# Wangshihu12/colmap-pcd

Hardware: AMD Instinct MI355X
Metric: NN queries/sec + BA-iter ms, 10M-pt cloud / 1M 3D feats (higher is better)
Workload: dtype f32 (NN distances) / f64 (association, BA); 1 GPU; M: 10000000-pt 'planes' cloud / 1000000 queries + BA scene 1000 cams / 1000000 pts / 4721253 obs / 900000 lidar terms (OPENCV), the same total at every N; cloud_points=10000000, queries=1000000, queries_this_rank=1000000, parallelism=single GPU

## Files before the change

colmap-pcd_amd/csrc/ba.hip:

```cpp
#include <algorithm>
#include <chrono>
#include <cmath>
#include <limits>
#include <memory>
#include <numeric>

#include "ba_cam_jac.h"
#include "ba_math.h"
#include "common.h"

namespace pcd {

struct BaDev {
  const int* cam_model; const int* cam_off; const double* cam_params;
  const double* poses; const int* image_cam; const uint8_t* image_const_pose; const uint8_t* image_const_tvec;
  const double* points; const uint8_t* point_const;
  const int* obs_image; const int* obs_point; const double* obs_xy;
  const int* lidar_point; const double* lidar_abcd; const double* lidar_w;
  const int* pt_order;
  const uint32_t* slice_start;
  const int* sell_img;
  const double* sell_xy;
  const uint32_t* pt_lidar_start; const uint32_t* pt_lidar_list;
  const uint32_t* img_obs_start;
  const int* img_pt;
  const uint32_t* img_obs;
  const uint32_t* seg_img;
  const uint32_t* seg_begin;
  const uint32_t* img_seg_start;
  const uint8_t* cam_refine;
  const uint32_t* cam_img_start;
  const uint32_t* cam_img_list;
  int C;
  int cam_k;
  const double* img_xy;
  int I, P, nslices; uint64_t O, L;
  int loss_type; double loss_scale;
};

template <int MODEL>
__device__ __forceinline__ void eval_block(const BaDev& d, int im, const double X[3], double ox, double oy,
                                           ReprojBlock& b, double q[4]) {
  const double* pose = d.poses + 7 * (size_t)im;
  double t[3];
#pragma unroll
  for (int k = 0; k < 4; ++k) q[k] = pose[k];
#pragma unroll
  for (int k = 0; k < 3; ++k) t[k] = pose[4 + k];
  const int cm = d.image_cam[im];
  const int model = MODEL >= 0 ? MODEL : d.cam_model[cm];
  reproj_eval(model, d.cam_params + d.cam_off[cm], q, t, X, ox, oy, b);
}

template <int N>
__device__ __forceinline__ void wave_store_rows(double* __restrict__ out, uint64_t row0, int cnt, const double (&v)[N],
                                                double* __restrict__ lds) {
  static_assert(N % 2 == 0, "rows are moved in 16-byte units");
  const int lane = threadIdx.x & 63;
#pragma unroll
  for (int k = 0; k < N; ++k) lds[lane * N + k] = v[k];
  __builtin_amdgcn_fence(__ATOMIC_RELEASE, "workgroup");
  __builtin_amdgcn_wave_barrier();
  __builtin_amdgcn_fence(__ATOMIC_ACQUIRE, "workgroup");
  const double2* src = reinterpret_cast<const double2*>(lds);
  double2* dst = reinterpret_cast<double2*>(out + row0 * N);
  const int units = cnt * (N / 2);
#pragma unroll
  for (int j = 0; j < N / 2; ++j) {
    const int u = j * 64 + lane;
    if (u < units) dst[u] = src[u];
  }
  __builtin_amdgcn_fence(__ATOMIC_RELEASE, "workgroup");
  __builtin_amdgcn_wave_barrier();
}

template <int MODEL, bool BLOCKS>
__global__ __launch_bounds__(256) void k_ba_points(BaDev d, double* __restrict__ Hpt, double* __restrict__ gpt,
                                                   double* __restrict__ cost_partial) {
  __shared__ double s_half[2][64][9];
  const int sl = threadIdx.x >> 7, half = (threadIdx.x >> 6) & 1, lane = threadIdx.x & 63;
  const int slice = blockIdx.x * 2 + sl;
  const int t = slice * 64 + lane;
  double cost = 0.0;
  double H[6] = {0, 0, 0, 0, 0, 0}, g[3] = {0, 0, 0};
  int p = -1;
  bool cpt = true;
  double X[3] = {0, 0, 0};
  if (slice < d.nslices) {
    p = d.pt_order[t];
    const uint32_t s0 = d.slice_start[slice], s1 = d.slice_start[slice + 1];
    if (p >= 0) {
      X[0] = d.points[3 * (size_t)p]; X[1] = d.points[3 * (size_t)p + 1]; X[2] = d.points[3 * (size_t)p + 2];
      cpt = d.point_const && d.point_const[p];
    }
    for (uint32_t s = s0 + lane + 64u * half; s < s1; s += 128) {
      const int im = d.sell_img[s];
      if (im < 0) continue;
      ReprojBlock b;
      double q[4];
      eval_block<MODEL>(d, im, X, d.sell_xy[2 * (size_t)s], d.sell_xy[2 * (size_t)s + 1], b, q);
      double rho0, rho1;
      loss_eval(d.loss_type, d.loss_scale, b.r[0] * b.r[0] + b.r[1] * b.r[1], rho0, rho1);
      cost += 0.5 * rho0;
      if (BLOCKS && !cpt) {
        const double sr = sqrt(rho1);
        double J[6];
#pragma unroll
        for (int r = 0; r < 2; ++r)
#pragma unroll
          for (int k = 0; k < 3; ++k)
            J[3 * r + k] = sr * (b.M[3 * r] * b.D[k] + b.M[3 * r + 1] * b.D[3 + k] + b.M[3 * r + 2] * b.D[6 + k]);
        const double r0 = sr * b.r[0], r1 = sr * b.r[1];
        H[0] += J[0] * J[0] + J[3] * J[3]; H[1] += J[0] * J[1] + J[3] * J[4]; H[2] += J[0] * J[2] + J[3] * J[5];
        H[3] += J[1] * J[1] + J[4] * J[4]; H[4] += J[1] * J[2] + J[4] * J[5]; H[5] += J[2] * J[2] + J[5] * J[5];
        g[0] += J[0] * r0 + J[3] * r1; g[1] += J[1] * r0 + J[4] * r1; g[2] += J[2] * r0 + J[5] * r1;
      }
    }
  }
  if (BLOCKS && half == 1) {
#pragma unroll
    for (int k = 0; k < 6; ++k) s_half[sl][lane][k] = H[k];
#pragma unroll
    for (int k = 0; k < 3; ++k) s_half[sl][lane][6 + k] = g[k];
  }
  __syncthreads();
  if (half == 0 && slice < d.nslices) {
    if (BLOCKS) {
#pragma unroll
      for (int k = 0; k < 6; ++k) H[k] += s_half[sl][lane][k];
#pragma unroll
      for (int k = 0; k < 3; ++k) g[k] += s_half[sl][lane][6 + k];
    }
    if (p >= 0) {
      for (uint32_t e = d.pt_lidar_start[p]; e < d.pt_lidar_start[p + 1]; ++e) {
        const uint32_t l = d.pt_lidar_list[e];
        const double abcd[4] = {d.lidar_abcd[4 * (size_t)l], d.lidar_abcd[4 * (size_t)l + 1],
                                d.lidar_abcd[4 * (size_t)l + 2], d.lidar_abcd[4 * (size_t)l + 3]};
        double r, J[3];
        lidar_eval(X, abcd, d.lidar_w[l], 0, r, J);
        double rho0, rho1;
        loss_eval(d.loss_type, d.loss_scale, r * r, rho0, rho1);
        cost += 0.5 * rho0;
        if (BLOCKS && !cpt) {
          const double sr = sqrt(rho1);
          const double rc = sr * r;
          J[0] *= sr; J[1] *= sr; J[2] *= sr;
          H[0] += J[0] * J[0]; H[1] += J[0] * J[1]; H[2] += J[0] * J[2];
          H[3] += J[1] * J[1]; H[4] += J[1] * J[2]; H[5] += J[2] * J[2];
          g[0] += J[0] * rc; g[1] += J[1] * rc; g[2] += J[2] * rc;
        }
      }
      if (BLOCKS && Hpt) {
        double* h = Hpt + 9 * (size_t)p;
        h[0] = H[0]; h[1] = H[1]; h[2] = H[2]; h[3] = H[1]; h[4] = H[3]; h[5] = H[4]; h[6] = H[2]; h[7] = H[4]; h[8] = H[5];
      }
      if (BLOCKS && gpt) { gpt[3 * (size_t)p] = g[0]; gpt[3 * (size_t)p + 1] = g[1]; gpt[3 * (size_t)p + 2] = g[2]; }
    }
  }
  __syncthreads();
  __shared__ double s_c[256];
  s_c[threadIdx.x] = cost;
  __syncthreads();
  for (int off = 128; off > 0; off >>= 1) {
    if ((int)threadIdx.x < off) s_c[threadIdx.x] += s_c[threadIdx.x + off];
    __syncthreads();
  }
  if (threadIdx.x == 0) cost_partial[blockIdx.x] = s_c[0];
}

template <int MODEL>
__global__ __launch_bounds__(256) void k_ba_cost(BaDev d, double* __restrict__ cost_partial) {
  double cost = 0.0;
  for (uint64_t i = blockIdx.x * (uint64_t)256 + threadIdx.x; i < d.O + d.L; i += (uint64_t)gridDim.x * 256) {
    if (i < d.O) {
      const int im = d.obs_image[i], pt = d.obs_point[i];
      const double X[3] = {d.points[3 * (size_t)pt], d.points[3 * (size_t)pt + 1], d.points[3 * (size_t)pt + 2]};
      ReprojBlock b;
      double q[4];
      eval_block<MODEL>(d, im, X, d.obs_xy[2 * i], d.obs_xy[2 * i + 1], b, q);
      double rho0, rho1;
      loss_eval(d.loss_type, d.loss_scale, b.r[0] * b.r[0] + b.r[1] * b.r[1], rho0, rho1);
      cost += 0.5 * rho0;
    } else {
      const uint64_t l = i - d.O;
      const int pt = d.lidar_point[l];
      const double X[3] = {d.points[3 * (size_t)pt], d.points[3 * (size_t)pt + 1], d.points[3 * (size_t)pt + 2]};
      const double abcd[4] = {d.lidar_abcd[4 * l], d.lidar_abcd[4 * l + 1], d.lidar_abcd[4 * l + 2], d.lidar_abcd[4 * l + 3]};
      double r, J[3];
      lidar_eval(X, abcd, d.lidar_w[l], 0, r, J);
      double rho0, rho1;
      loss_eval(d.loss_type, d.loss_scale, r * r, rho0, rho1);
      cost += 0.5 * rho0;
    }
  }
  __shared__ double s_c[256];
  s_c[threadIdx.x] = cost;
  __syncthreads();
  for (int off = 128; off > 0; off >>= 1) {
    if ((int)threadIdx.x < off) s_c[threadIdx.x] += s_c[threadIdx.x + off];
    __syncthreads();
  }
  if (threadIdx.x == 0) cost_partial[blockIdx.x] = s_c[0];
}
constexpr unsigned kCostBlocks = 1u << 20;

__global__ __launch_bounds__(256) void k_sum_partials(const double* __restrict__ partial, int n, double* __restrict__ out) {
  __shared__ double s_c[256];
  double a0 = 0.0, a1 = 0.0, a2 = 0.0, a3 = 0.0;
  int i = threadIdx.x;
  for (; i + 768 < n; i += 1024) { a0 += partial[i]; a1 += partial[i + 256]; a2 += partial[i + 512]; a3 += partial[i + 768]; }
  for (; i < n; i += 256) a0 += partial[i];
  s_c[threadIdx.x] = (a0 + a1) + (a2 + a3);
  __syncthreads();
  for (int off = 128; off > 0; off >>= 1) {
    if ((int)threadIdx.x < off) s_c[threadIdx.x] += s_c[threadIdx.x + off];
    __syncthreads();
  }
  if (threadIdx.x == 0) out[0] = s_c[0];
}

constexpr uint32_t kImgSeg = 1024;
template <int MODEL, bool WANT_W>
__global__ __launch_bounds__(256) void k_ba_images(BaDev d, double* __restrict__ partial, double* __restrict__ W_o) {
  __shared__ __attribute__((aligned(16))) double s_w[WANT_W ? 4 : 1][WANT_W ? 64 * 18 : 2];
  const int im = (int)d.seg_img[blockIdx.x];
  const int lane = threadIdx.x & 63;
  const int wave = __builtin_amdgcn_readfirstlane((int)(threadIdx.x >> 6));
  const bool cpose = d.image_const_pose && d.image_const_pose[im];
  double acc[27];
#pragma unroll
  for (int k = 0; k < 27; ++k) acc[k] = 0.0;
  const unsigned tmask = d.image_const_tvec ? d.image_const_tvec[im] : 0u;
  const uint32_t e_beg = d.seg_begin[blockIdx.x];
  const uint32_t e_end = min(d.seg_begin[blockIdx.x + 1], d.img_obs_start[im + 1]);
  if (!cpose || WANT_W) {
    for (uint32_t e0 = e_beg; e0 < e_end; e0 += 256) {
      const uint32_t e = e0 + threadIdx.x;
      const bool active = e < e_end;
      double w[18];
#pragma unroll
      for (int k = 0; k < 18; ++k) w[k] = 0.0;
      if (active && !cpose) {
        const int pt = d.img_pt[e];
        const double X[3] = {d.points[3 * (size_t)pt], d.points[3 * (size_t)pt + 1], d.points[3 * (size_t)pt + 2]};
        ReprojBlock b;
        double q[4];
        eval_block<MODEL>(d, im, X, d.img_xy[2 * (size_t)e], d.img_xy[2 * (size_t)e + 1], b, q);
        double rho0, rho1;
        loss_eval(d.loss_type, d.loss_scale, b.r[0] * b.r[0] + b.r[1] * b.r[1], rho0, rho1);
        const double sr = sqrt(rho1);
        double Jq[8], Jt[6], JX[6], Jqt[6];
        reproj_jacobians(b, Jq, Jt, JX);
        quat_tangent(q, Jq, Jqt);
        double J[12];
#pragma unroll
        for (int r = 0; r < 2; ++r)
#pragma unroll
          for (int k = 0; k < 3; ++k) {
            J[6 * r + k] = sr * Jqt[3 * r + k];
            J[6 * r + 3 + k] = ((tmask >> k) & 1u) ? 0.0 : sr * Jt[3 * r + k];
          }
        const double r0 = sr * b.r[0], r1 = sr * b.r[1];
        int idx = 0;
#pragma unroll
        for (int a = 0; a < 6; ++a)
#pragma unroll
          for (int c = a; c < 6; ++c) acc[idx++] += J[a] * J[c] + J[6 + a] * J[6 + c];
#pragma unroll
        for (int a = 0; a < 6; ++a) acc[21 + a] += J[a] * r0 + J[6 + a] * r1;
        if (WANT_W && !(d.point_const && d.point_const[pt])) {
#pragma unroll
          for (int a = 0; a < 6; ++a)
#pragma unroll
            for (int c = 0; c < 3; ++c) w[3 * a + c] = J[a] * (sr * JX[c]) + J[6 + a] * (sr * JX[3 + c]);
        }
      }
      if (WANT_W) {
        const uint32_t o = active ? d.img_obs[e] : 0u;
        const uint32_t o_first = (uint32_t)__builtin_amdgcn_readfirstlane((int)o);
        const int cnt = (int)min(64u, e_end > e0 + wave * 64u ? e_end - (e0 + wave * 64u) : 0u);
        const bool contiguous = __all(!active || o == o_first + (uint32_t)lane);
        if (contiguous) {
          wave_store_rows<18>(W_o, o_first, cnt, w, s_w[wave]);
        } else if (active) {
          double* dst = W_o + 18 * (size_t)o;
#pragma unroll
          for (int k = 0; k < 18; ++k) dst[k] = w[k];
        }
      }
    }
  }
  __shared__ double s_a[4][27];
#pragma unroll
  for (int k = 0; k < 27; ++k) {
    double v = acc[k];
#pragma unroll
    for (int off = 32; off > 0; off >>= 1) v += __shfl_xor(v, off);
    if (lane == 0) s_a[wave][k] = v;
  }
  __syncthreads();
  if (threadIdx.x < 27)
    partial[27 * (size_t)blockIdx.x + threadIdx.x] =
        (s_a[0][threadIdx.x] + s_a[1][threadIdx.x]) + (s_a[2][threadIdx.x] + s_a[3][threadIdx.x]);
}

__global__ __launch_bounds__(64) void k_ba_images_reduce(BaDev d, const double* __restrict__ partial,
                                                         double* __restrict__ Himg, double* __restrict__ gimg) {
  const int im = blockIdx.x * 2 + (threadIdx.x >> 5), k = threadIdx.x & 31;
  if (im >= d.I || k >= 27) return;
  double v = 0.0;
  for (uint32_t sgm = d.img_seg_start[im]; sgm < d.img_seg_start[im + 1]; ++sgm) v += partial[27 * (size_t)sgm + k];
  if (k >= 21) {
    if (gimg) gimg[6 * (size_t)im + (k - 21)] = v;
  } else if (Himg) {
    int a = 0, kk = k;
    while (kk >= 6 - a) { kk -= 6 - a; ++a; }
    const int c = a + kk;
    Himg[36 * (size_t)im + 6 * a + c] = v;
    Himg[36 * (size_t)im + 6 * c + a] = v;
  }
}

__host__ __device__ constexpr int cam_ne(int K) { return K * (K + 1) / 2 + 6 * K + K; }
__host__ __device__ constexpr int cam_ent_l(int K, int e) {
  const int ncc = K * (K + 1) / 2;
  if (e < ncc) { int a = 0; while (e >= K - a) { e -= K - a; ++a; } return a; }
  e -= ncc;
  if (e < 6 * K) return e / 6;
  return e - 6 * K;
}
__host__ __device__ constexpr int cam_ent_r(int K, int e) {
  const int ncc = K * (K + 1) / 2;
  if (e < ncc) { int a = 0; while (e >= K - a) { e -= K - a; ++a; } return a + e; }
  e -= ncc;
  if (e < 6 * K) return K + e % 6;
  return K + 6;
}

template <int MODEL, int CH>
__device__ __forceinline__ void cam_accumulate(const BaDev& d, int im, double* __restrict__ partial) {
  constexpr int K = MODEL >= 0 ? cam_num_params(MODEL >= 0 ? MODEL : 0) : PCD_CAM_JAC_STRIDE;
  constexpr int NE = cam_ne(K), PER = (NE + 3) / 4, E0 = CH * PER, E1 = E0 + PER < NE ? E0 + PER : NE;
  constexpr int NA = K + 7;
  const int lane = threadIdx.x & 63;
  const bool cpose = d.image_const_pose && d.image_const_pose[im];
  const unsigned tmask = d.image_const_tvec ? d.image_const_tvec[im] : 0u;
  const int cm = d.image_cam[im];
  const double* cam = d.cam_params + d.cam_off[cm];
  const uint8_t* refine = d.cam_refine ? d.cam_refine + d.cam_off[cm] : nullptr;
  const int model = MODEL >= 0 ? MODEL : d.cam_model[cm];
  double acc[PER > 0 ? PER : 1];
#pragma unroll
  for (int t = 0; t < PER; ++t) acc[t] = 0.0;
  for (uint32_t e = d.img_obs_start[im] + lane; e < d.img_obs_start[im + 1]; e += 64) {
    const int pt = d.img_pt[e];
    const double X[3] = {d.points[3 * (size_t)pt], d.points[3 * (size_t)pt + 1], d.points[3 * (size_t)pt + 2]};
    ReprojBlock b;
    double q[4];
    eval_block<MODEL>(d, im, X, d.img_xy[2 * (size_t)e], d.img_xy[2 * (size_t)e + 1], b, q);
    double rho0, rho1;
    loss_eval(d.loss_type, d.loss_scale, b.r[0] * b.r[0] + b.r[1] * b.r[1], rho0, rho1);
    const double sr = sqrt(rho1);
    double A[2][NA];
    {
      const double* pose = d.poses + 7 * (size_t)im;
      const double w = pose[0], a = pose[1], bq = pose[2], c = pose[3];
      const double cx = bq * X[2] - c * X[1], cy = c * X[0] - a * X[2], cz = a * X[1] - bq * X[0];
      const double ux = 2.0 * cx, uy = 2.0 * cy, uz = 2.0 * cz;
      const double Px = X[0] + w * ux + (bq * uz - c * uy) + pose[4];
      const double Py = X[1] + w * uy + (c * ux - a * uz) + pose[5];
      const double Pz = X[2] + w * uz + (a * uy - bq * ux) + pose[6];
      const double iz = 1.0 / Pz;
      double Jc[2 * K];
#pragma unroll
      for (int k = 0; k < 2 * K; ++k) Jc[k] = 0.0;
      if (MODEL >= 0) cam_param_jacobian<(MODEL >= 0 ? MODEL : 0)>(cam, Px * iz, Py * iz, Jc, K);
      else cam_param_jacobian_any(model, cam, Px * iz, Py * iz, Jc, K);
      const int kn = MODEL >= 0 ? K : cam_num_params(model);
#pragma unroll
      for (int k = 0; k < K; ++k) {
        const bool var = refine && k < kn && refine[k < kn ? k : 0];
        A[0][k] = var ? sr * Jc[k] : 0.0;
        A[1][k] = var ? sr * Jc[K + k] : 0.0;
      }
    }
    double Jq[8], Jt[6], JX[6], Jqt[6];
    reproj_jacobians(b, Jq, Jt, JX);
    quat_tangent(q, Jq, Jqt);
#pragma unroll
    for (int r = 0; r < 2; ++r) {
// ... 1332 lines not shown
      b->nseg = (uint32_t)seg_img.size();
      seg_begin.push_back((uint32_t)b->O);
      UP(seg_img, seg_img.data(), seg_img.size());
      UP(seg_begin, seg_begin.data(), seg_begin.size());
      UP(img_seg_start, img_seg_start.data(), img_seg_start.size());
    }
    {
      std::vector<uint32_t> cst, cli;
      build_csr(d->image_camera, (uint64_t)b->I, b->C, cst, cli);
      UP(cam_img_start, cst.data(), cst.size());
      UP(cam_img_list, cli.data(), cli.size());
    }
    UP(img_obs, li.data(), li.size());
    pcd_status sa = b->img_pt.reserve(std::max<size_t>(b->O, 1));
    if (sa == PCD_OK) sa = b->img_xy.reserve(std::max<size_t>(2 * b->O, 2));
    if (sa != PCD_OK) return fail(sa);
    if (b->O)
      hipLaunchKernelGGL(k_ba_fill_image_major, dim3(div_up(b->O, 256)), dim3(256), 0, nullptr, b->img_obs.p,
                         b->obs_point.p, b->obs_xy.p, b->O, b->img_pt.p, b->img_xy.p);
    if (hipDeviceSynchronize() != hipSuccess || hipGetLastError() != hipSuccess) {
      set_error("pcd_ba_create: filling the image-major layout failed");
      return fail(PCD_ERR_HIP);
    }
  }
#undef UP
  {
    b->h_pose_row.assign(b->O, 0xFFFFFFFFu);
    std::vector<uint32_t> vobs;
    vobs.reserve(b->O);
    for (uint64_t o = 0; o < b->O; ++o)
      if (!(d->image_const_pose && d->image_const_pose[d->obs_image[o]])) {
        b->h_pose_row[o] = (uint32_t)vobs.size();
        vobs.push_back((uint32_t)o);
      }
    b->n_pose_rows = vobs.size();
    if (b->n_pose_rows != b->O) {
      pcd_status sv = upload(b->vobs, vobs.data(), vobs.size());
      if (sv != PCD_OK) return fail(sv);
    }
  }
  pcd_status s1 = b->cost_partial.reserve((size_t)std::max(cost_blocks(b, true), cost_blocks(b, false)) + 1);
  if (s1 != PCD_OK) return fail(s1);
  if ((s1 = b->cost.reserve(1)) != PCD_OK) return fail(s1);
  *out = b;
  return PCD_OK;
  });
}

void pcd_ba_destroy(pcd_ba* b) {
  if (!b) return;
  (void)hipSetDevice(b->device);
  delete b;
}

pcd_status pcd_ba_set_parameters(pcd_ba* b, const double* poses, const double* points) {
  PCD_REQUIRE(b, "null handle");
  PCD_HIP_TRY(hipSetDevice(b->device));
  if (poses) PCD_HIP_TRY(hipMemcpy(b->poses.p, poses, 7 * (size_t)b->I * sizeof(double), hipMemcpyHostToDevice));
  if (points) PCD_HIP_TRY(hipMemcpy(b->points.p, points, 3 * (size_t)b->P * sizeof(double), hipMemcpyHostToDevice));
  return PCD_OK;
}

pcd_status pcd_ba_set_camera_parameters(pcd_ba* b, const double* cam_params) {
  PCD_REQUIRE(b && cam_params, "null pointer");
  PCD_HIP_TRY(hipSetDevice(b->device));
  PCD_HIP_TRY(hipMemcpy(b->cam_params.p, cam_params, b->cam_params_len * sizeof(double), hipMemcpyHostToDevice));
  return PCD_OK;
}

pcd_status pcd_ba_device_parameters(pcd_ba* b, double** d_poses, double** d_points) {
  PCD_REQUIRE(b, "null handle");
  if (d_poses) *d_poses = b->poses.p;
  if (d_points) *d_points = b->points.p;
  return PCD_OK;
}

pcd_status pcd_ba_evaluate_device(pcd_ba* b, const pcd_ba_out* o, void* stream) {
  PCD_REQUIRE(b && o, "null pointer");
  PCD_REFUSE_CAPTURE(stream);
  PCD_HIP_TRY(hipSetDevice(b->device));
  hipStream_t s = (hipStream_t)stream;
  const BaDev d = b->dev();
  const int model = b->uniform_model;
  if (o->cost || o->H_pt || o->g_pt) {
    const bool want_blocks = o->H_pt || o->g_pt;
    const unsigned blocks = cost_blocks(b, want_blocks);
    {
      ScopedKernelTimer t(want_blocks ? "ba_points" : "ba_points_cost", s);
      if (want_blocks) {
        PCD_BA_DISPATCH(model, hipLaunchKernelGGL((k_ba_points<M, true>), dim3(blocks), dim3(256), 0, s, d, o->H_pt,
                                                   o->g_pt, b->cost_partial.p));
      } else {
        PCD_BA_DISPATCH(model, hipLaunchKernelGGL((k_ba_cost<M>), dim3(blocks), dim3(256), 0, s, d, b->cost_partial.p));
      }
    }
    if (o->cost) hipLaunchKernelGGL(k_sum_partials, dim3(1), dim3(256), 0, s, b->cost_partial.p, (int)blocks, o->cost);
  }
  const bool w_fused = o->W && (o->H_img || o->g_img) && b->O;
  if (o->H_img || o->g_img) {
    PCD_TRY(b->img_partial.reserve(27 * (size_t)std::max(b->nseg, 1u)));
    ScopedKernelTimer t(w_fused ? "ba_images_w" : "ba_images", s);
    if (b->nseg) {
      if (w_fused) {
        PCD_BA_DISPATCH(model, hipLaunchKernelGGL((k_ba_images<M, true>), dim3(b->nseg), dim3(256), 0, s, d,
                                                   b->img_partial.p, o->W));
      } else {
        PCD_BA_DISPATCH(model, hipLaunchKernelGGL((k_ba_images<M, false>), dim3(b->nseg), dim3(256), 0, s, d,
                                                   b->img_partial.p, (double*)nullptr));
      }
    }
    hipLaunchKernelGGL(k_ba_images_reduce, dim3(div_up(b->I, 2)), dim3(64), 0, s, d, b->img_partial.p, o->H_img, o->g_img);
  }
  double* const W_raw = w_fused ? nullptr : o->W;
  if ((o->residuals || o->jac_q || o->jac_t || o->jac_X || W_raw) && b->O) {
    ScopedKernelTimer t("ba_raw", s);
    PCD_BA_DISPATCH(model, hipLaunchKernelGGL((k_ba_raw<M>), dim3(div_up(b->O, 256)), dim3(256), 0, s, d, o->residuals,
                                               o->jac_q, o->jac_t, o->jac_X, W_raw));
  }
  if (o->jac_cam && b->O) {
    ScopedKernelTimer t("ba_cam_jac", s);
    PCD_BA_DISPATCH(model, hipLaunchKernelGGL((k_ba_cam_jac<M>), dim3(div_up(b->O, 256)), dim3(256), 0, s, d, o->jac_cam));
  }
  if (o->H_cam || o->g_cam || o->E_cam) {
    PCD_TRY(b->cam_partial.reserve((size_t)b->I * cam_ne(PCD_CAM_JAC_STRIDE)));
    ScopedKernelTimer t("ba_cameras", s);
    PCD_BA_DISPATCH(model, hipLaunchKernelGGL((k_ba_cameras<M>), dim3(b->I), dim3(256), 0, s, d, b->cam_partial.p));
    hipLaunchKernelGGL(k_ba_cameras_reduce, dim3(b->C), dim3(256), 0, s, d, b->cam_partial.p, o->H_cam, o->g_cam,
                       o->E_cam);
  }
  if (o->W_cam && b->O) {
    ScopedKernelTimer t("ba_cam_w", s);
    PCD_BA_DISPATCH(model, hipLaunchKernelGGL((k_ba_cam_w<M>), dim3(div_up(b->O, 256)), dim3(256), 0, s, d, o->W_cam));
  }
  if ((o->residuals || o->jac_lidar) && b->L) {
    ScopedKernelTimer t("ba_lidar_raw", s);
    hipLaunchKernelGGL(k_ba_lidar_raw, dim3(div_up(b->L, 256)), dim3(256), 0, s, d, o->residuals, o->jac_lidar);
  }
  PCD_HIP_TRY(hipGetLastError());
  return PCD_OK;
}

pcd_status pcd_ba_observation_errors_device(pcd_ba* b, double* d_sq_err, double* d_depth, void* stream) {
  PCD_REQUIRE(b, "null handle");
  PCD_REFUSE_CAPTURE(stream);
  if (!b->O || (!d_sq_err && !d_depth)) return PCD_OK;
  PCD_HIP_TRY(hipSetDevice(b->device));
  hipStream_t s = (hipStream_t)stream;
  const BaDev d = b->dev();
  const int model = b->uniform_model;
  ScopedKernelTimer t("ba_obs_errors", s);
  PCD_BA_DISPATCH(model, hipLaunchKernelGGL((k_ba_obs_errors<M>), dim3(div_up(b->O, 256)), dim3(256), 0, s, d, d_sq_err,
                                            d_depth));
  PCD_HIP_TRY(hipGetLastError());
  return PCD_OK;
}

pcd_status pcd_ba_observation_errors(pcd_ba* b, double* sq_err, double* depth) {
  PCD_REQUIRE(b, "null handle");
  if (!b->O) return PCD_OK;
  PCD_HIP_TRY(hipSetDevice(b->device));
  PCD_TRY(b->o_jq.reserve(b->O));
  PCD_TRY(b->o_jt.reserve(b->O));
  PCD_TRY(pcd_ba_observation_errors_device(b, sq_err ? b->o_jq.p : nullptr, depth ? b->o_jt.p : nullptr, nullptr));
  if (sq_err) PCD_HIP_TRY(hipMemcpy(sq_err, b->o_jq.p, b->O * sizeof(double), hipMemcpyDeviceToHost));
  if (depth) PCD_HIP_TRY(hipMemcpy(depth, b->o_jt.p, b->O * sizeof(double), hipMemcpyDeviceToHost));
  return PCD_OK;
}

pcd_status pcd_ba_filter_tracks_device(pcd_ba* b, double max_reproj_error, const pcd_ba_filter_out* o, void* stream) {
  PCD_REQUIRE(b && o, "null pointer");
  PCD_REFUSE_CAPTURE(stream);
  PCD_HIP_TRY(hipSetDevice(b->device));
  hipStream_t s = (hipStream_t)stream;
  const uint64_t O = b->O;
  const int nbp = (int)div_up((uint64_t)b->P, 256), nbo = (int)div_up(std::max<uint64_t>(O, 1), 256);
  PCD_TRY(b->f_sq.reserve(std::max<uint64_t>(O, 1))); PCD_TRY(b->f_depth.reserve(std::max<uint64_t>(O, 1)));
  PCD_TRY(b->f_part.reserve(3 * (size_t)nbp + nbo + 4));
  if (O) PCD_TRY(pcd_ba_observation_errors_device(b, b->f_sq.p, b->f_depth.p, s));
  ScopedKernelTimer t("ba_filter_tracks", s);
  double* part3 = b->f_part.p, *part1 = b->f_part.p + 3 * (size_t)nbp;
  hipLaunchKernelGGL(k_ba_filter_tracks, dim3(nbp), dim3(256), 0, s, b->P, b->pt_obs_start.p, b->pt_obs_list.p, b->f_sq.p,
                     max_reproj_error * max_reproj_error, o->obs_erase, o->point_delete, o->point_error, part3);
  hipLaunchKernelGGL(k_ba_negative_depth, dim3(nbo), dim3(256), 0, s, O, b->f_depth.p, o->obs_negative_depth, part1);
  if (o->summary) hipLaunchKernelGGL(k_ba_filter_summary, dim3(1), dim3(256), 0, s, part3, nbp, part1, nbo, o->summary);
  PCD_HIP_TRY(hipGetLastError());
  return PCD_OK;
}

pcd_status pcd_ba_filter_tracks(pcd_ba* b, double max_reproj_error, const pcd_ba_filter_out* o) {
  PCD_REQUIRE(b && o, "null pointer");
  PCD_HIP_TRY(hipSetDevice(b->device));
  const size_t O = b->O, P = (size_t)b->P;
  PCD_TRY(b->f_u8.reserve(2 * O + P + 1)); PCD_TRY(b->f_summary.reserve(P + 4));
  pcd_ba_filter_out d{};
// ... 90 lines not shown
    }
  PCD_TRY(pcd_ba_evaluate_device(b, &d, nullptr));
  for (auto& it : items)
    if (it.host && it.n) PCD_HIP_TRY(hipMemcpy(it.host, it.buf->p, it.n * sizeof(double), hipMemcpyDeviceToHost));
  PCD_HIP_TRY(hipDeviceSynchronize());
  return PCD_OK;
}

pcd_status pcd_ba_schur_structure(pcd_ba* b, int32_t* image_slot, int32_t* num_slots, uint64_t* num_pairs,
                                  int32_t* pair_i, int32_t* pair_j) {
  return pcd::guard([&]() -> pcd_status {
    PCD_TRY(schur_guard(b));
    PCD_TRY(schur_build(b));
    const BaSchur& S = *b->schur;
    if (image_slot) std::memcpy(image_slot, S.h_slot.data(), (size_t)b->I * sizeof(int32_t));
    if (num_slots) *num_slots = S.ns;
    if (num_pairs) *num_pairs = S.npairs;
    if (pair_i && S.npairs) std::memcpy(pair_i, S.h_pair_i.data(), S.npairs * sizeof(int32_t));
    if (pair_j && S.npairs) std::memcpy(pair_j, S.h_pair_j.data(), S.npairs * sizeof(int32_t));
    return PCD_OK;
  });
}

pcd_status pcd_ba_schur_stats(pcd_ba* b, pcd_ba_schur_info* info) {
  PCD_TRY(schur_guard(b));
  PCD_REQUIRE(info, "null pointer");
  std::memset(info, 0, sizeof *info);
  if (!b->schur || !b->schur->built) return PCD_OK;
  const BaSchur& S = *b->schur;
  info->build_ms = S.build_ms;
  info->num_entries = S.nent;
  uint64_t bytes = 0;
  bytes += (S.img_slot.n + S.slot_img.n) * sizeof(int);
  bytes += (S.blk_start.n + S.ent_a.n + S.ent_b.n + S.pair_ij.n + S.iota.n + S.obs_pos.n + S.skip_partial.n +
            S.row_start.n + S.row_blk.n + S.row_col.n) * sizeof(uint32_t);
  for (const DevBuf<double>* d : {&S.Himg, &S.gimg, &S.Hpt, &S.gpt, &S.Wim, &S.Y, &S.Vinv, &S.Vg, &S.Dpt, &S.Dimg,
                                  &S.Sdiag, &S.Soff, &S.rhs, &S.md_partial, &S.md, &S.cost, &S.dense,
                                  &S.Minv, &S.cg_x0, &S.cg_x1, &S.cg_r, &S.cg_z, &S.cg_p0, &S.cg_p1, &S.cg_w, &S.cg_pw,
                                  &S.cg_partial, &S.cg_out, &S.lm_dpose, &S.lm_dpoint, &S.lm_poses, &S.lm_points,
                                  &S.lm_cand_cost, &S.lm_gpart})
    bytes += d->n * sizeof(double);
  bytes += S.cg_state.n * sizeof(PcgState) + S.cg_info.n * sizeof(pcd_ba_pcg_info) + S.lm_rec.n * sizeof(LmRecord);
  info->scratch_bytes = bytes;
  return PCD_OK;
}

pcd_status pcd_ba_schur_device(pcd_ba* b, const pcd_ba_schur_opts* opt, const pcd_ba_schur_out* o, void* stream) {
  return pcd::guard([&]() -> pcd_status {
    PCD_TRY(schur_guard(b));
    PCD_REQUIRE(opt && o, "null pointer");
    PCD_REQUIRE(opt->damping == PCD_DAMP_MARQUARDT || opt->damping == PCD_DAMP_LEVENBERG, "damping");
    PCD_REQUIRE(opt->mu >= 0.0, "mu must be >= 0");
    PCD_REFUSE_CAPTURE(stream);
    PCD_TRY(schur_build(b));
    BaSchur& S = *b->schur;
    hipStream_t s = (hipStream_t)stream;
    const int I = b->I, P = b->P, ns = S.ns;
    const uint64_t O = b->O;
    const uint32_t nblk = (uint32_t)(ns + S.npairs);
    const unsigned nbp = std::max(1u, div_up((uint64_t)P, 256));
    S.valid = false;
    PCD_TRY(S.Himg.reserve(36 * (size_t)I)); PCD_TRY(S.gimg.reserve(6 * (size_t)I));
    PCD_TRY(S.Hpt.reserve(9 * (size_t)P)); PCD_TRY(S.gpt.reserve(3 * (size_t)P));
    PCD_TRY(S.Wim.reserve(std::max<size_t>(18 * O, 1))); PCD_TRY(S.Y.reserve(std::max<size_t>(18 * O, 1)));
    PCD_TRY(S.Vinv.reserve(9 * (size_t)P)); PCD_TRY(S.Vg.reserve(3 * (size_t)P)); PCD_TRY(S.Dpt.reserve(3 * (size_t)P));
    PCD_TRY(S.Dimg.reserve(std::max<size_t>(6 * (size_t)ns, 1)));
    PCD_TRY(S.Sdiag.reserve(std::max<size_t>(36 * (size_t)ns, 1)));
    PCD_TRY(S.Soff.reserve(std::max<size_t>(36 * S.npairs, 1)));
    PCD_TRY(S.rhs.reserve(std::max<size_t>(6 * (size_t)ns, 1)));
    PCD_TRY(S.skip_partial.reserve(nbp)); PCD_TRY(S.skip_cnt.reserve(1));
    PCD_TRY(S.md_partial.reserve(nbp)); PCD_TRY(S.md.reserve(1)); PCD_TRY(S.cost.reserve(1));
    PCD_TRY(b->img_partial.reserve(27 * (size_t)std::max(b->nseg, 1u)));
    PCD_HIP_TRY(hipSetDevice(b->device));
    const BaDev d = b->dev();
    BaDev dim = d;
    dim.img_obs = S.iota.p;
    const int model = b->uniform_model;
    double* Sdiag = o->S_diag ? o->S_diag : S.Sdiag.p;
    double* Soff = o->S_off ? o->S_off : S.Soff.p;
    double* rhs = o->rhs ? o->rhs : S.rhs.p;
    {
      ScopedKernelTimer t("ba_schur_normal", s);
      const unsigned blocks = cost_blocks(b, true);
      PCD_BA_DISPATCH(model, hipLaunchKernelGGL((k_ba_points<M, true>), dim3(blocks), dim3(256), 0, s, d, S.Hpt.p,
                                                 S.gpt.p, b->cost_partial.p));
      hipLaunchKernelGGL(k_sum_partials, dim3(1), dim3(256), 0, s, b->cost_partial.p, (int)blocks,
                         o->cost ? o->cost : S.cost.p);
      if (b->nseg)
        PCD_BA_DISPATCH(model, hipLaunchKernelGGL((k_ba_images<M, true>), dim3(b->nseg), dim3(256), 0, s, dim,
                                                   b->img_partial.p, S.Wim.p));
      hipLaunchKernelGGL(k_ba_images_reduce, dim3(div_up(I, 2)), dim3(64), 0, s, d, b->img_partial.p, S.Himg.p, S.gimg.p);
    }
    {
      ScopedKernelTimer t("ba_schur_eliminate", s);
      hipLaunchKernelGGL(k_schur_points, dim3(nbp), dim3(256), 0, s, P, S.Hpt.p, S.gpt.p, d.point_const, opt->mu,
                         opt->damping, S.Vinv.p, S.Vg.p, S.Dpt.p, S.skip_partial.p);
      hipLaunchKernelGGL(k_sum_u32, dim3(1), dim3(256), 0, s, S.skip_partial.p, (int)nbp,
                         o->num_skipped ? reinterpret_cast<unsigned long long*>(o->num_skipped) : S.skip_cnt.p);
      if (O) hipLaunchKernelGGL(k_schur_obs, dim3(div_up(O, 256)), dim3(256), 0, s, O, b->img_pt.p, S.Wim.p, S.Vinv.p, S.Y.p);
      SchurBlocks sb;
      sb.ns = ns; sb.nblk = nblk; sb.blk_start = S.blk_start.p; sb.ent_a = S.ent_a.p; sb.ent_b = S.ent_b.p;
      sb.pair_ij = S.pair_ij.p; sb.slot_img = S.slot_img.p; sb.img_obs_start = b->img_obs_start.p; sb.img_pt = b->img_pt.p;
      sb.Y = S.Y.p; sb.Wim = S.Wim.p; sb.Vg = S.Vg.p; sb.Himg = S.Himg.p; sb.gimg = S.gimg.p;
      sb.image_const_tvec = d.image_const_tvec; sb.mu = opt->mu; sb.mode = opt->damping;
      sb.Sdiag = Sdiag; sb.Soff = Soff; sb.rhs = rhs; sb.Dimg = S.Dimg.p;
      if (nblk) hipLaunchKernelGGL(k_schur_blocks, dim3(div_up(nblk, 4)), dim3(256), 0, s, sb);
    }
    if (o->S && ns) {
      ScopedKernelTimer t("ba_schur_dense", s);
      const size_t n = 6 * (size_t)ns;
      PCD_HIP_TRY(hipMemsetAsync(o->S, 0, n * n * sizeof(double), s));
      hipLaunchKernelGGL(k_schur_dense, dim3(div_up((uint64_t)nblk * 36, 256)), dim3(256), 0, s, ns, nblk, S.pair_ij.p,
                         Sdiag, Soff, o->S);
    }
    PCD_HIP_TRY(hipGetLastError());
    S.valid = true;
    S.own_diag = !o->S_diag; S.own_off = !o->S_off; S.own_rhs = !o->rhs;
    return PCD_OK;
  });
}

pcd_status pcd_ba_schur(pcd_ba* b, const pcd_ba_schur_opts* opt, const pcd_ba_schur_out* o) {
  return pcd::guard([&]() -> pcd_status {
    PCD_TRY(schur_guard(b));
    PCD_REQUIRE(opt && o, "null pointer");
    PCD_TRY(schur_build(b));
    BaSchur& S = *b->schur;
    const size_t n = 6 * (size_t)S.ns;
    pcd_ba_schur_out d{};
    if (o->S) { PCD_TRY(S.dense.reserve(std::max<size_t>(n * n, 1))); d.S = S.dense.p; }
    PCD_TRY(pcd_ba_schur_device(b, opt, &d, nullptr));
    if (o->cost) PCD_HIP_TRY(hipMemcpy(o->cost, S.cost.p, sizeof(double), hipMemcpyDeviceToHost));
    if (o->num_skipped) PCD_HIP_TRY(hipMemcpy(o->num_skipped, S.skip_cnt.p, sizeof(uint64_t), hipMemcpyDeviceToHost));
    if (o->S_diag && S.ns) PCD_HIP_TRY(hipMemcpy(o->S_diag, S.Sdiag.p, 36 * (size_t)S.ns * sizeof(double), hipMemcpyDeviceToHost));
    if (o->S_off && S.npairs) PCD_HIP_TRY(hipMemcpy(o->S_off, S.Soff.p, 36 * S.npairs * sizeof(double), hipMemcpyDeviceToHost));
    if (o->rhs && S.ns) PCD_HIP_TRY(hipMemcpy(o->rhs, S.rhs.p, 6 * (size_t)S.ns * sizeof(double), hipMemcpyDeviceToHost));
    if (o->S && n) PCD_HIP_TRY(hipMemcpy(o->S, S.dense.p, n * n * sizeof(double), hipMemcpyDeviceToHost));
    PCD_HIP_TRY(hipDeviceSynchronize());
    return PCD_OK;
  });
}

pcd_status pcd_ba_schur_back_substitute_device(pcd_ba* b, const double* d_dpose, double* d_dpoint,
                                               double* d_model_decrease, void* stream) {
  PCD_TRY(schur_guard(b));
  PCD_REFUSE_CAPTURE(stream);
  if (!b->schur || !b->schur->valid) {
    set_error("pcd_ba_schur_back_substitute_device: no Schur state (call pcd_ba_schur[_device] first)");
    return PCD_ERR_INVALID;
  }
  BaSchur& S = *b->schur;
  PCD_REQUIRE((d_dpose || S.ns == 0) && (d_dpoint || b->P == 0), "null pointer");
  PCD_HIP_TRY(hipSetDevice(b->device));
  hipStream_t s = (hipStream_t)stream;
  const int P = b->P;
  const unsigned nbp = std::max(1u, div_up((uint64_t)P, 256));
  ScopedKernelTimer t("ba_schur_back", s);
  hipLaunchKernelGGL(k_schur_back, dim3(nbp), dim3(256), 0, s, P, b->pt_obs_start.p, b->pt_obs_list.p, b->obs_image.p,
                     S.obs_pos.p, S.img_slot.p, S.Wim.p, S.Vinv.p, S.gpt.p, S.Dpt.p, d_dpose, d_dpoint, S.md_partial.p);
  if (d_model_decrease)
    hipLaunchKernelGGL(k_schur_model_decrease, dim3(1), dim3(256), 0, s, S.ns, S.slot_img.p,
                       b->has_ctvec ? b->image_const_tvec.p : (const uint8_t*)nullptr, S.gimg.p, S.Dimg.p, d_dpose,
                       S.md_partial.p, (int)nbp, d_model_decrease);
  PCD_HIP_TRY(hipGetLastError());
  return PCD_OK;
}

pcd_status pcd_ba_plus_device(pcd_ba* b, const double* d_dpose, const double* d_dpoint, double* d_poses_out,
                              double* d_points_out, void* stream) {
  return pcd::guard([&]() -> pcd_status {
    PCD_TRY(schur_guard(b));
    PCD_REFUSE_CAPTURE(stream);
    PCD_TRY(schur_build(b));
    PCD_REQUIRE((d_dpose || b->schur->ns == 0) && (d_dpoint || b->P == 0) && (d_poses_out || b->I == 0) &&
// ... 292 lines not shown
```

Baseline: 739.4 million queries/s.

## Use f64 MFMA for image normal blocks and widen point kernel to four waves

The per-image kernel now stages each observation's Jacobian rows and residuals in LDS and accumulates the 6x6 normal block plus gradient with f64 16x16x4 MFMA, replacing 27 per-lane scalar accumulators and their shuffle reductions. It also software-prefetches the next observation's inputs. The per-point kernel moves to 512 threads, four waves per slice, reducing per-round terms through LDS with block barriers. The separate cost-sum launch is folded into an extra block of the image-reduce kernel to save a launch. The trade-offs are more LDS traffic and barriers, MFMA work on padded 16x16 tiles, and waves-per-EU hints that change register pressure.

After: 723.8 million queries/s. -2.1%, worse.

```diff
diff --git a/colmap-pcd_amd/csrc/ba.hip b/colmap-pcd_amd/csrc/ba.hip
--- a/colmap-pcd_amd/csrc/ba.hip
+++ b/colmap-pcd_amd/csrc/ba.hip
@@ -52,6 +52,12 @@
   reproj_eval(model, d.cam_params + d.cam_off[cm], q, t, X, ox, oy, b);
 }
 
+#if defined(PCD_ABLATE) && defined(PCD_BA_ABLATE)
+constexpr int kBaAblate = PCD_BA_ABLATE;
+#else
+constexpr int kBaAblate = 0;
+#endif
+
 template <int N>
 __device__ __forceinline__ void wave_store_rows(double* __restrict__ out, uint64_t row0, int cnt, const double (&v)[N],
                                                 double* __restrict__ lds) {
@@ -75,61 +81,89 @@
 }
 
 template <int MODEL, bool BLOCKS>
-__global__ __launch_bounds__(256) void k_ba_points(BaDev d, double* __restrict__ Hpt, double* __restrict__ gpt,
+__global__ __launch_bounds__(512) __attribute__((amdgpu_waves_per_eu(MODEL >= 0 ? 4 : 1))) void k_ba_points(BaDev d, double* __restrict__ Hpt, double* __restrict__ gpt,
                                                    double* __restrict__ cost_partial) {
-  __shared__ double s_half[2][64][9];
-  const int sl = threadIdx.x >> 7, half = (threadIdx.x >> 6) & 1, lane = threadIdx.x & 63;
+  constexpr int NT = BLOCKS ? 10 : 1;
+  __shared__ double s_t[2][4][NT][64];
+  __shared__ double s_c[256];
+  const int sl = threadIdx.x >> 8, wv = (threadIdx.x >> 6) & 3, lane = threadIdx.x & 63;
   const int slice = blockIdx.x * 2 + sl;
   const int t = slice * 64 + lane;
-  double cost = 0.0;
-  double H[6] = {0, 0, 0, 0, 0, 0}, g[3] = {0, 0, 0};
   int p = -1;
   bool cpt = true;
   double X[3] = {0, 0, 0};
+  uint32_t s0 = 0, s1 = 0;
   if (slice < d.nslices) {
     p = d.pt_order[t];
-    const uint32_t s0 = d.slice_start[slice], s1 = d.slice_start[slice + 1];
+    s0 = d.slice_start[slice]; s1 = d.slice_start[slice + 1];
     if (p >= 0) {
       X[0] = d.points[3 * (size_t)p]; X[1] = d.points[3 * (size_t)p + 1]; X[2] = d.points[3 * (size_t)p + 2];
       cpt = d.point_const && d.point_const[p];
     }
-    for (uint32_t s = s0 + lane + 64u * half; s < s1; s += 128) {
-      const int im = d.sell_img[s];
-      if (im < 0) continue;
+  }
+  uint32_t rows = 0;
+#pragma unroll
+  for (int k = 0; k < 2; ++k) {
+    const int sk = blockIdx.x * 2 + k;
+    if (sk < d.nslices) rows = max(rows, (d.slice_start[sk + 1] - d.slice_start[sk]) >> 6);
+  }
+  const uint32_t nrounds = (rows + 3) >> 2;
+  __shared__ double s_acc[2][2][NT][64];
+  if (wv == 0) {
+#pragma unroll
+    for (int c = 0; c < 2; ++c)
+#pragma unroll
+      for (int k = 0; k < NT; ++k) s_acc[sl][c][k][lane] = 0.0;
+  }
+  for (uint32_t r = 0; r < nrounds; ++r) {
+    const uint32_t s = s0 + 64u * (4u * r + (uint32_t)wv) + (uint32_t)lane;
+    double term[NT];
+#pragma unroll
+    for (int k = 0; k < NT; ++k) term[k] = 0.0;
+    const int im = s < s1 ? d.sell_img[s] : -1;
+    if (im >= 0) {
       ReprojBlock b;
       double q[4];
       eval_block<MODEL>(d, im, X, d.sell_xy[2 * (size_t)s], d.sell_xy[2 * (size_t)s + 1], b, q);
       double rho0, rho1;
       loss_eval(d.loss_type, d.loss_scale, b.r[0] * b.r[0] + b.r[1] * b.r[1], rho0, rho1);
-      cost += 0.5 * rho0;
+      term[NT - 1] = 0.5 * rho0;
       if (BLOCKS && !cpt) {
         const double sr = sqrt(rho1);
         double J[6];
 #pragma unroll
-        for (int r = 0; r < 2; ++r)
+        for (int rr = 0; rr < 2; ++rr)
 #pragma unroll
           for (int k = 0; k < 3; ++k)
-            J[3 * r + k] = sr * (b.M[3 * r] * b.D[k] + b.M[3 * r + 1] * b.D[3 + k] + b.M[3 * r + 2] * b.D[6 + k]);
+            J[3 * rr + k] = sr * (b.M[3 * rr] * b.D[k] + b.M[3 * rr + 1] * b.D[3 + k] + b.M[3 * rr + 2] * b.D[6 + k]);
         const double r0 = sr * b.r[0], r1 = sr * b.r[1];
-        H[0] += J[0] * J[0] + J[3] * J[3]; H[1] += J[0] * J[1] + J[3] * J[4]; H[2] += J[0] * J[2] + J[3] * J[5];
-        H[3] += J[1] * J[1] + J[4] * J[4]; H[4] += J[1] * J[2] + J[4] * J[5]; H[5] += J[2] * J[2] + J[5] * J[5];
-        g[0] += J[0] * r0 + J[3] * r1; g[1] += J[1] * r0 + J[4] * r1; g[2] += J[2] * r0 + J[5] * r1;
-      }
-    }
-  }
-  if (BLOCKS && half == 1) {
-#pragma unroll
-    for (int k = 0; k < 6; ++k) s_half[sl][lane][k] = H[k];
-#pragma unroll
-    for (int k = 0; k < 3; ++k) s_half[sl][lane][6 + k] = g[k];
-  }
-  __syncthreads();
-  if (half == 0 && slice < d.nslices) {
+        term[0] = J[0] * J[0] + J[3] * J[3]; term[1] = J[0] * J[1] + J[3] * J[4]; term[2] = J[0] * J[2] + J[3] * J[5];
+        term[3] = J[1] * J[1] + J[4] * J[4]; term[4] = J[1] * J[2] + J[4] * J[5]; term[5] = J[2] * J[2] + J[5] * J[5];
+        term[6] = J[0] * r0 + J[3] * r1; term[7] = J[1] * r0 + J[4] * r1; term[8] = J[2] * r0 + J[5] * r1;
+      }
+    }
+    if (r) __syncthreads();
+#pragma unroll
+    for (int k = 0; k < NT; ++k) s_t[sl][wv][k][lane] = term[k];
+    __syncthreads();
+    if (wv == 0) {
+#pragma unroll
+      for (int c = 0; c < 2; ++c)
+#pragma unroll
+        for (int k = 0; k < NT; ++k)
+          s_acc[sl][c][k][lane] = (s_acc[sl][c][k][lane] + s_t[sl][c][k][lane]) + s_t[sl][c + 2][k][lane];
+    }
+    if (kBaAblate & 4) break;
+  }
+  double c0 = 0.0, c1 = 0.0;
+  if (wv == 0 && slice < d.nslices) {
+    double H[6] = {0, 0, 0, 0, 0, 0}, g[3] = {0, 0, 0};
+    c0 = s_acc[sl][0][NT - 1][lane]; c1 = s_acc[sl][1][NT - 1][lane];
     if (BLOCKS) {
 #pragma unroll
-      for (int k = 0; k < 6; ++k) H[k] += s_half[sl][lane][k];
-#pragma unroll
-      for (int k = 0; k < 3; ++k) g[k] += s_half[sl][lane][6 + k];
+      for (int k = 0; k < 6; ++k) H[k] = s_acc[sl][0][k][lane] + s_acc[sl][1][k][lane];
+#pragma unroll
+      for (int k = 0; k < 3; ++k) g[k] = s_acc[sl][0][6 + k][lane] + s_acc[sl][1][6 + k][lane];
     }
     if (p >= 0) {
       for (uint32_t e = d.pt_lidar_start[p]; e < d.pt_lidar_start[p + 1]; ++e) {
@@ -140,7 +174,7 @@
         lidar_eval(X, abcd, d.lidar_w[l], 0, r, J);
         double rho0, rho1;
         loss_eval(d.loss_type, d.loss_scale, r * r, rho0, rho1);
-        cost += 0.5 * rho0;
+        c0 += 0.5 * rho0;
         if (BLOCKS && !cpt) {
           const double sr = sqrt(rho1);
           const double rc = sr * r;
@@ -157,9 +191,7 @@
       if (BLOCKS && gpt) { gpt[3 * (size_t)p] = g[0]; gpt[3 * (size_t)p + 1] = g[1]; gpt[3 * (size_t)p + 2] = g[2]; }
     }
   }
-  __syncthreads();
-  __shared__ double s_c[256];
-  s_c[threadIdx.x] = cost;
+  if (wv == 0) { s_c[sl * 128 + lane] = c0; s_c[sl * 128 + 64 + lane] = c1; }
   __syncthreads();
   for (int off = 128; off > 0; off >>= 1) {
     if ((int)threadIdx.x < off) s_c[threadIdx.x] += s_c[threadIdx.x + off];
@@ -220,39 +252,72 @@
 }
 
 constexpr uint32_t kImgSeg = 1024;
+constexpr int kImgRow = 15;
+
+struct ImgObsIn {
+  int pt; uint32_t o; bool pconst;
+  double X[3], ox, oy;
+};
+template <bool WANT_W>
+__device__ __forceinline__ void img_obs_load(const BaDev& d, uint32_t e, bool active, bool want_point, ImgObsIn& in) {
+  in.pt = 0; in.o = 0u; in.pconst = false;
+  in.X[0] = in.X[1] = in.X[2] = in.ox = in.oy = 0.0;
+  if (!active) return;
+  if (WANT_W) in.o = d.img_obs[e];
+  if (!want_point) return;
+  in.pt = d.img_pt[e];
+  in.ox = d.img_xy[2 * (size_t)e]; in.oy = d.img_xy[2 * (size_t)e + 1];
+  in.X[0] = d.points[3 * (size_t)in.pt]; in.X[1] = d.points[3 * (size_t)in.pt + 1]; in.X[2] = d.points[3 * (size_t)in.pt + 2];
+  if (WANT_W) in.pconst = d.point_const && d.point_const[in.pt];
+}
+
+typedef double ba_f64x4 __attribute__((ext_vector_type(4)));
+
 template <int MODEL, bool WANT_W>
-__global__ __launch_bounds__(256) void k_ba_images(BaDev d, double* __restrict__ partial, double* __restrict__ W_o) {
-  __shared__ __attribute__((aligned(16))) double s_w[WANT_W ? 4 : 1][WANT_W ? 64 * 18 : 2];
+__global__ __launch_bounds__(256) __attribute__((amdgpu_waves_per_eu(MODEL >= 0 ? 4 : 1))) void k_ba_images(BaDev d, double* __restrict__ partial, double* __restrict__ W_o) {
+  constexpr int kScratch = WANT_W ? 64 * 18 : 64 * kImgRow;
+  static_assert(kScratch >= 64 * kImgRow && kScratch >= 256, "rows of 64 observations, then the 16x16 result");
+  __shared__ __attribute__((aligned(16))) double s_w[4][kScratch];
   const int im = (int)d.seg_img[blockIdx.x];
   const int lane = threadIdx.x & 63;
   const int wave = __builtin_amdgcn_readfirstlane((int)(threadIdx.x >> 6));
   const bool cpose = d.image_const_pose && d.image_const_pose[im];
-  double acc[27];
-#pragma unroll
-  for (int k = 0; k < 27; ++k) acc[k] = 0.0;
+  ba_f64x4 acc = {0.0, 0.0, 0.0, 0.0};
   const unsigned tmask = d.image_const_tvec ? d.image_const_tvec[im] : 0u;
   const uint32_t e_beg = d.seg_begin[blockIdx.x];
   const uint32_t e_end = min(d.seg_begin[blockIdx.x + 1], d.img_obs_start[im + 1]);
+  double* const lds = s_w[wave];
+  const double* const mrow = lds + (2 * (lane >> 5) + ((lane >> 3) & 1)) * kImgRow + ((lane >> 4) & 1) * 7 + min(lane & 7, 6);
+  constexpr bool kPrefetch = !(kBaAblate & 2);
   if (!cpose || WANT_W) {
+    ImgObsIn nxt;
+    if (kPrefetch) img_obs_load<WANT_W>(d, e_beg + threadIdx.x, e_beg + threadIdx.x < e_end, !cpose, nxt);
     for (uint32_t e0 = e_beg; e0 < e_end; e0 += 256) {
       const uint32_t e = e0 + threadIdx.x;
       const bool active = e < e_end;
+      ImgObsIn in;
+      if (kPrefetch) {
+        in = nxt;
+        img_obs_load<WANT_W>(d, e + 256, e + 256 < e_end, !cpose, nxt);
+      } else {
+        img_obs_load<WANT_W>(d, e, active, !cpose, in);
+      }
       double w[18];
 #pragma unroll
       for (int k = 0; k < 18; ++k) w[k] = 0.0;
+      double J[12], r0 = 0.0, r1 = 0.0;
+#pragma unroll
+      for (int k = 0; k < 12; ++k) J[k] = 0.0;
       if (active && !cpose) {
-        const int pt = d.img_pt[e];
-        const double X[3] = {d.points[3 * (size_t)pt], d.points[3 * (size_t)pt + 1], d.points[3 * (size_t)pt + 2]};
         ReprojBlock b;
         double q[4];
-        eval_block<MODEL>(d, im, X, d.img_xy[2 * (size_t)e], d.img_xy[2 * (size_t)e + 1], b, q);
+        eval_block<MODEL>(d, im, in.X, in.ox, in.oy, b, q);
         double rho0, rho1;
         loss_eval(d.loss_type, d.loss_scale, b.r[0] * b.r[0] + b.r[1] * b.r[1], rho0, rho1);
         const double sr = sqrt(rho1);
         double Jq[8], Jt[6], JX[6], Jqt[6];
         reproj_jacobians(b, Jq, Jt, JX);
         quat_tangent(q, Jq, Jqt);
-        double J[12];
 #pragma unroll
         for (int r = 0; r < 2; ++r)
 #pragma unroll
@@ -260,28 +325,40 @@
             J[6 * r + k] = sr * Jqt[3 * r + k];
             J[6 * r + 3 + k] = ((tmask >> k) & 1u) ? 0.0 : sr * Jt[3 * r + k];
           }
-        const double r0 = sr * b.r[0], r1 = sr * b.r[1];
-        int idx = 0;
-#pragma unroll
-        for (int a = 0; a < 6; ++a)
-#pragma unroll
-          for (int c = a; c < 6; ++c) acc[idx++] += J[a] * J[c] + J[6 + a] * J[6 + c];
-#pragma unroll
-        for (int a = 0; a < 6; ++a) acc[21 + a] += J[a] * r0 + J[6 + a] * r1;
-        if (WANT_W && !(d.point_const && d.point_const[pt])) {
+        r0 = sr * b.r[0]; r1 = sr * b.r[1];
+        if (WANT_W && !in.pconst) {
 #pragma unroll
           for (int a = 0; a < 6; ++a)
 #pragma unroll
             for (int c = 0; c < 3; ++c) w[3 * a + c] = J[a] * (sr * JX[c]) + J[6 + a] * (sr * JX[3 + c]);
         }
       }
+      if (kBaAblate & 1) {
+#pragma unroll
+        for (int k = 0; k < 12; ++k) asm volatile("" ::"v"(J[k]));
+        asm volatile("" ::"v"(r0), "v"(r1));
+      } else if (!cpose) {
+#pragma unroll
+        for (int k = 0; k < 6; ++k) { lds[lane * kImgRow + k] = J[k]; lds[lane * kImgRow + 7 + k] = J[6 + k]; }
+        lds[lane * kImgRow + 6] = r0; lds[lane * kImgRow + 13] = r1;
+        __builtin_amdgcn_fence(__ATOMIC_RELEASE, "workgroup");
+        __builtin_amdgcn_wave_barrier();
+        __builtin_amdgcn_fence(__ATOMIC_ACQUIRE, "workgroup");
+#pragma unroll
+        for (int m = 0; m < 16; ++m) {
+          const double v = mrow[m * 4 * kImgRow];
+          acc = __builtin_amdgcn_mfma_f64_16x16x4f64(v, v, acc, 0, 0, 0);
+        }
+        __builtin_amdgcn_fence(__ATOMIC_RELEASE, "workgroup");
+        __builtin_amdgcn_wave_barrier();
+      }
       if (WANT_W) {
-        const uint32_t o = active ? d.img_obs[e] : 0u;
+        const uint32_t o = in.o;
         const uint32_t o_first = (uint32_t)__builtin_amdgcn_readfirstlane((int)o);
         const int cnt = (int)min(64u, e_end > e0 + wave * 64u ? e_end - (e0 + wave * 64u) : 0u);
         const bool contiguous = __all(!active || o == o_first + (uint32_t)lane);
         if (contiguous) {
-          wave_store_rows<18>(W_o, o_first, cnt, w, s_w[wave]);
+          wave_store_rows<18>(W_o, o_first, cnt, w, lds);
         } else if (active) {
           double* dst = W_o + 18 * (size_t)o;
 #pragma unroll
@@ -290,22 +367,56 @@
       }
     }
   }
-  __shared__ double s_a[4][27];
-#pragma unroll
-  for (int k = 0; k < 27; ++k) {
-    double v = acc[k];
-#pragma unroll
-    for (int off = 32; off > 0; off >>= 1) v += __shfl_xor(v, off);
-    if (lane == 0) s_a[wave][k] = v;
-  }
+#pragma unroll
+  for (int j = 0; j < 4; ++j) lds[((lane >> 4) + 4 * j) * 16 + (lane & 15)] = acc[j];
   __syncthreads();
-  if (threadIdx.x < 27)
-    partial[27 * (size_t)blockIdx.x + threadIdx.x] =
-        (s_a[0][threadIdx.x] + s_a[1][threadIdx.x]) + (s_a[2][threadIdx.x] + s_a[3][threadIdx.x]);
+  if (threadIdx.x < 27) {
+    int a, c;
+    if (threadIdx.x >= 21) { a = threadIdx.x - 21; c = 6; }
+    else { a = 0; int kk = threadIdx.x; while (kk >= 6 - a) { kk -= 6 - a; ++a; } c = a + kk; }
+    double v[4];
+#pragma unroll
+    for (int wv = 0; wv < 4; ++wv) v[wv] = s_w[wv][a * 16 + c] + s_w[wv][(8 + a) * 16 + 8 + c];
+    partial[27 * (size_t)blockIdx.x + threadIdx.x] = (v[0] + v[1]) + (v[2] + v[3]);
+  }
 }
 
 __global__ __launch_bounds__(64) void k_ba_images_reduce(BaDev d, const double* __restrict__ partial,
-                                                         double* __restrict__ Himg, double* __restrict__ gimg) {
+                                                         double* __restrict__ Himg, double* __restrict__ gimg,
+                                                         const double* __restrict__ cost_partial, int ncost,
+                                                         double* __restrict__ cost_out) {
+  if (cost_out && blockIdx.x == gridDim.x - 1) {
+    __shared__ double s_c[256];
+    double a[4][4];
+#pragma unroll
+    for (int v = 0; v < 4; ++v)
+#pragma unroll
+      for (int k = 0; k < 4; ++k) a[v][k] = 0.0;
+    int i = threadIdx.x;
+    for (; i + 192 + 768 < ncost; i += 1024) {
+#pragma unroll
+      for (int v = 0; v < 4; ++v)
+#pragma unroll
+        for (int k = 0; k < 4; ++k) a[v][k] += cost_partial[i + 64 * v + 256 * k];
+    }
+#pragma unroll
+    for (int v = 0; v < 4; ++v) {
+      int iv = i + 64 * v;
+      for (; iv + 768 < ncost; iv += 1024) {
+#pragma unroll
+        for (int k = 0; k < 4; ++k) a[v][k] += cost_partial[iv + 256 * k];
+      }
+      for (; iv < ncost; iv += 256) a[v][0] += cost_partial[iv];
+      s_c[threadIdx.x + 64 * v] = (a[v][0] + a[v][1]) + (a[v][2] + a[v][3]);
+    }
+    __syncthreads();
+    for (int off = 128; off > 0; off >>= 1) {
+      for (int t = threadIdx.x; t < off; t += 64) s_c[t] += s_c[t + off];
+      __syncthreads();
+    }
+    if (threadIdx.x == 0) cost_out[0] = s_c[0];
+    return;
+  }
   const int im = blockIdx.x * 2 + (threadIdx.x >> 5), k = threadIdx.x & 31;
   if (im >= d.I || k >= 27) return;
   double v = 0.0;
@@ -1804,19 +1915,24 @@
   hipStream_t s = (hipStream_t)stream;
   const BaDev d = b->dev();
   const int model = b->uniform_model;
+  bool cost_in_reduce = false;
+  int ncost = 0;
   if (o->cost || o->H_pt || o->g_pt) {
     const bool want_blocks = o->H_pt || o->g_pt;
     const unsigned blocks = cost_blocks(b, want_blocks);
     {
       ScopedKernelTimer t(want_blocks ? "ba_points" : "ba_points_cost", s);
       if (want_blocks) {
-        PCD_BA_DISPATCH(model, hipLaunchKernelGGL((k_ba_points<M, true>), dim3(blocks), dim3(256), 0, s, d, o->H_pt,
+        PCD_BA_DISPATCH(model, hipLaunchKernelGGL((k_ba_points<M, true>), dim3(blocks), dim3(512), 0, s, d, o->H_pt,
                                                    o->g_pt, b->cost_partial.p));
       } else {
         PCD_BA_DISPATCH(model, hipLaunchKernelGGL((k_ba_cost<M>), dim3(blocks), dim3(256), 0, s, d, b->cost_partial.p));
       }
     }
-    if (o->cost) hipLaunchKernelGGL(k_sum_partials, dim3(1), dim3(256), 0, s, b->cost_partial.p, (int)blocks, o->cost);
+    cost_in_reduce = o->cost && want_blocks && (o->H_img || o->g_img);
+    ncost = (int)blocks;
+    if (o->cost && !cost_in_reduce)
+      hipLaunchKernelGGL(k_sum_partials, dim3(1), dim3(256), 0, s, b->cost_partial.p, (int)blocks, o->cost);
   }
   const bool w_fused = o->W && (o->H_img || o->g_img) && b->O;
   if (o->H_img || o->g_img) {
@@ -1831,7 +1947,9 @@
                                                    b->img_partial.p, (double*)nullptr));
       }
     }
-    hipLaunchKernelGGL(k_ba_images_reduce, dim3(div_up(b->I, 2)), dim3(64), 0, s, d, b->img_partial.p, o->H_img, o->g_img);
+    hipLaunchKernelGGL(k_ba_images_reduce, dim3(div_up(b->I, 2) + (cost_in_reduce ? 1 : 0)), dim3(64), 0, s, d,
+                       b->img_partial.p, o->H_img, o->g_img, b->cost_partial.p, ncost,
+                       cost_in_reduce ? o->cost : (double*)nullptr);
   }
   double* const W_raw = w_fused ? nullptr : o->W;
   if ((o->residuals || o->jac_q || o->jac_t || o->jac_X || W_raw) && b->O) {
@@ -2088,14 +2206,13 @@
     {
       ScopedKernelTimer t("ba_schur_normal", s);
       const unsigned blocks = cost_blocks(b, true);
-      PCD_BA_DISPATCH(model, hipLaunchKernelGGL((k_ba_points<M, true>), dim3(blocks), dim3(256), 0, s, d, S.Hpt.p,
+      PCD_BA_DISPATCH(model, hipLaunchKernelGGL((k_ba_points<M, true>), dim3(blocks), dim3(512), 0, s, d, S.Hpt.p,
                                                  S.gpt.p, b->cost_partial.p));
-      hipLaunchKernelGGL(k_sum_partials, dim3(1), dim3(256), 0, s, b->cost_partial.p, (int)blocks,
-                         o->cost ? o->cost : S.cost.p);
       if (b->nseg)
         PCD_BA_DISPATCH(model, hipLaunchKernelGGL((k_ba_images<M, true>), dim3(b->nseg), dim3(256), 0, s, dim,
                                                    b->img_partial.p, S.Wim.p));
-      hipLaunchKernelGGL(k_ba_images_reduce, dim3(div_up(I, 2)), dim3(64), 0, s, d, b->img_partial.p, S.Himg.p, S.gimg.p);
+      hipLaunchKernelGGL(k_ba_images_reduce, dim3(div_up(I, 2) + 1), dim3(64), 0, s, d, b->img_partial.p, S.Himg.p,
+                         S.gimg.p, b->cost_partial.p, (int)blocks, o->cost ? o->cost : S.cost.p);
     }
     {
       ScopedKernelTimer t("ba_schur_eliminate", s);
```
